# wolfbox/snappy

Hardware: AMD Instinct MI355X
Metric: GiB/s hashed (whole node), bit-exact hashes.yaml, 10k x 1 MiB tree (higher is better)
Workload: dtype u64; 1 GPU; C2: ONE on-disk tree (tmpfs) of 10001 files (10 000 x 1 MiB + the 1 MiB archive stand-in) -> hashes.yaml, sharded over 1 rank(s) on 1 distinct GPU(s); bytes=10486808576, kernel=sha512_split_kernel<true>, tree_home=/dev/shm

## Files before the change

snappy_amd/csrc/hostfill.cpp:

```cpp
#include "hostfill.h"

#include <new>

#include <ctype.h>
#include <dirent.h>
#include <errno.h>
#include <sched.h>
#include <stdio.h>
#include <string.h>
#include <sys/syscall.h>
#include <unistd.h>

#include <algorithm>
#include <atomic>

#if defined(__x86_64__)
#include <immintrin.h>
#endif

namespace snaphash {

namespace {

bool read_small_file(const std::string& path, std::string& out)
// ... 103 lines not shown
}

int numa_node_of_address(const void* addr)
{
#if defined(SYS_get_mempolicy)
    int node = -1;
    if (syscall(SYS_get_mempolicy, &node, nullptr, 0ul, addr, (unsigned long)(kMpolFNode | kMpolFAddr)) != 0) return -1;
    return node;
#else
    (void)addr;
    return -1;
#endif
}

unsigned cgroup_cpu_quota(const std::string& sysfs_cgroup_root, const std::string& proc_self_cgroup)
{
    std::string text;
    if (!read_small_file(proc_self_cgroup, text)) return 0;
    double best = 0;
    auto take = [&](double quota, double period) {
        if (quota > 0 && period > 0) { const double c = quota / period; if (best == 0 || c < best) best = c; }
    };
    size_t pos = 0;
    while (pos < text.size()) {
        size_t eol = text.find('\n', pos);
        if (eol == std::string::npos) eol = text.size();
        const std::string line = text.substr(pos, eol - pos);
        pos = eol + 1;
        const size_t c1 = line.find(':'), c2 = c1 == std::string::npos ? c1 : line.find(':', c1 + 1);
        if (c2 == std::string::npos) continue;
        const std::string ctrl = line.substr(c1 + 1, c2 - c1 - 1);
        std::string path = line.substr(c2 + 1);
        const bool v2 = ctrl.empty();
        if (!v2) {
            bool has_cpu = false;
            for (size_t a = 0; a <= ctrl.size();) {
                size_t b = ctrl.find(',', a);
                if (b == std::string::npos) b = ctrl.size();
                if (ctrl.compare(a, b - a, "cpu") == 0) has_cpu = true;
                a = b + 1;
            }
            if (!has_cpu) continue;
        }
        const std::string base = sysfs_cgroup_root + (v2 ? "" : "/" + ctrl);
        for (;;) {
            std::string v;
            if (v2) {
                if (read_small_file(base + path + "/cpu.max", v) && v.compare(0, 3, "max") != 0) {
                    char* end = nullptr;
                    const double q = strtod(v.c_str(), &end);
                    const double per = end ? strtod(end, nullptr) : 0;
                    take(q, per);
                }
            } else {
                std::string pv;
                if (read_small_file(base + path + "/cpu.cfs_quota_us", v) && read_small_file(base + path + "/cpu.cfs_period_us", pv))
                    take(strtod(v.c_str(), nullptr), strtod(pv.c_str(), nullptr));
            }
            if (path.empty() || path == "/") break;
            const size_t slash = path.rfind('/');
            path = slash == 0 || slash == std::string::npos ? "/" : path.substr(0, slash);
        }
    }
    if (best <= 0) return 0;
    return (unsigned)std::max(1.0, best + 0.5);
}

unsigned usable_cpus()
{
    unsigned n = 0;
    cpu_set_t set;
    CPU_ZERO(&set);
    if (sched_getaffinity(0, sizeof set, &set) == 0) {
        const int c = CPU_COUNT(&set);
        if (c > 0) n = (unsigned)c;
    }
    if (n == 0) n = std::max(1u, std::thread::hardware_concurrency());
    static const unsigned quota = cgroup_cpu_quota("/sys/fs/cgroup", "/proc/self/cgroup");
    if (quota && quota < n) n = quota;
    return n;
}


FillPool::~FillPool() { stop(); }

void FillPool::stop()
{
    {
        std::lock_guard<std::mutex> lk(mu_);
        quit_ = true;
    }
    cv_work_.notify_all();
    for (auto& t : th_) if (t.joinable()) t.join();
    th_.clear();
    quit_ = false;
}

void FillPool::configure(unsigned max_threads, const std::vector<int>& cpus)
{
    stop();
    max_threads_ = max_threads;
    cpus_ = cpus;
}

void FillPool::worker(unsigned id)
{
    if (!cpus_.empty()) {
        cpu_set_t set, allowed;
        CPU_ZERO(&set);
        CPU_ZERO(&allowed);
        const bool have_allowed = sched_getaffinity(0, sizeof allowed, &allowed) == 0;
        for (int c : cpus_)
            if (c >= 0 && c < CPU_SETSIZE && (!have_allowed || CPU_ISSET(c, &allowed))) CPU_SET(c, &set);
        if (CPU_COUNT(&set) > 0) (void)sched_setaffinity(0, sizeof set, &set);
    }
    uint64_t seen = 0;
    for (;;) {
        const std::function<void(size_t)>* fn;
        size_t n;
        std::atomic<size_t>* next;
        {
            std::unique_lock<std::mutex> lk(mu_);
            cv_work_.wait(lk, [&] { return quit_ || (epoch_ != seen && id < want_); });
            if (quit_) return;
            seen = epoch_;
            fn = fn_; n = n_; next = next_;
        }
        try {
            for (;;) {
                const size_t i = next->fetch_add(1);
                if (i >= n) break;
                (*fn)(i);
            }
        } catch (...) {
            fn_threw_.store(true);
        }
        {
            std::lock_guard<std::mutex> lk(mu_);
            if (--running_ == 0) cv_done_.notify_all();
        }
    }
}

void FillPool::parallel_for(size_t n, unsigned threads, const std::function<void(size_t)>& fn)
{
    if (n == 0) return;
    unsigned helpers = threads > 1 ? std::min(threads - 1, max_threads_) : 0u;
    if (helpers > n - 1) helpers = (unsigned)(n - 1);
    std::atomic<size_t> next{0};
    if (helpers) {
        std::lock_guard<std::mutex> lk(mu_);
        try {
            while (th_.size() < helpers) { const unsigned id = (unsigned)th_.size(); th_.emplace_back(&FillPool::worker, this, id); }
        } catch (...) {
            helpers = (unsigned)th_.size();
        }
        if (helpers) {
            fn_ = &fn; n_ = n; next_ = &next;
            want_ = helpers;
            running_ = helpers;
            ++epoch_;
        }
    }
    if (helpers) cv_work_.notify_all();
    bool threw = false;
    try {
        for (;;) {
            const size_t i = next.fetch_add(1);
            if (i >= n) break;
            fn(i);
        }
    } catch (...) {
        threw = true;
        next.store(n);
    }
    if (helpers) {
        std::unique_lock<std::mutex> lk(mu_);
        cv_done_.wait(lk, [&] { return running_ == 0; });
        want_ = 0;
        fn_ = nullptr; next_ = nullptr;
    }
    if (fn_threw_.exchange(false) || threw) throw std::bad_alloc();
}


void run_on_threads(unsigned T, const std::function<void(unsigned)>& fn)
{
    if (T <= 1) { fn(0); return; }
    static std::mutex mu;
    static FillPool* pool = [] {
        FillPool* p = new FillPool();
        p->configure(64, {});
        return p;
    }();
    static const pid_t born_in = getpid();
    if (T <= 65 && getpid() == born_in && mu.try_lock()) {
        std::lock_guard<std::mutex> lk(mu, std::adopt_lock);
        pool->parallel_for(T, T, [&fn](size_t t) { fn((unsigned)t); });
// ... 41 lines not shown
```

snappy_amd/csrc/hostfill.h:

```cpp
#pragma once
#include <stddef.h>
#include <stdint.h>

#include <atomic>
#include <condition_variable>
#include <functional>
#include <mutex>
#include <new>
#include <string>
#include <thread>
#include <vector>

namespace snaphash {

int numa_node_of_pci(const std::string& sysfs_root, const std::string& bdf);
std::vector<int> numa_cpus_of_node(const std::string& sysfs_root, int node);
std::vector<int> parse_cpulist(const std::string& text);
int numa_node_count(const std::string& sysfs_root);
std::vector<int> slice_cpus(const std::vector<int>& all, size_t pos, size_t m);

struct SavedMemPolicy {
    bool valid = false;
    int mode = 0;
    unsigned long mask[1024 / (8 * sizeof(unsigned long)) + 1] = {0};
};
bool numa_prefer_node(int node, SavedMemPolicy* saved);
void numa_restore_policy(const SavedMemPolicy& saved);
int numa_node_of_address(const void* addr);
unsigned usable_cpus();
unsigned cgroup_cpu_quota(const std::string& sysfs_cgroup_root, const std::string& proc_self_cgroup);

struct ThreadJoiner {
    std::vector<std::thread> th;
    std::atomic<bool> worker_threw{false};
    ThreadJoiner() = default;
    ThreadJoiner(const ThreadJoiner&) = delete;
    ThreadJoiner& operator=(const ThreadJoiner&) = delete;
    ~ThreadJoiner() { join_quietly(); }
    template <class F, class... A> void spawn(F&& f, A&&... a)
    {
        th.emplace_back([this](auto fn, auto... args) {
            try { fn(args...); } catch (...) { worker_threw.store(true); }
        }, std::forward<F>(f), std::forward<A>(a)...);
    }
    void join_quietly()
    {
        for (auto& t : th)
            if (t.joinable()) t.join();
    }
    void join_all()
    {
        join_quietly();
        if (worker_threw.exchange(false)) throw std::bad_alloc();
    }
};

class FillPool {
public:
    FillPool() = default;
    ~FillPool();
    FillPool(const FillPool&) = delete;
    FillPool& operator=(const FillPool&) = delete;
    void configure(unsigned max_threads, const std::vector<int>& cpus);
    void parallel_for(size_t n, unsigned threads, const std::function<void(size_t)>& fn);
    unsigned max_threads() const { return max_threads_; }
    const std::vector<int>& cpus() const { return cpus_; }

private:
    void worker(unsigned id);
    void stop();
    unsigned max_threads_ = 0;
    std::vector<int> cpus_;
    std::vector<std::thread> th_;
    std::mutex mu_;
    std::condition_variable cv_work_, cv_done_;
    uint64_t epoch_ = 0;
    unsigned want_ = 0;
    unsigned running_ = 0;
    bool quit_ = false;
    const std::function<void(size_t)>* fn_ = nullptr;
    std::atomic<bool> fn_threw_{false};
    size_t n_ = 0;
    std::atomic<size_t>* next_ = nullptr;
};

void run_on_threads(unsigned T, const std::function<void(unsigned)>& fn);

void copy_to_staging(void* dst, const void* src, size_t n);

}
```

snappy_amd/csrc/snaphash_api.cpp:

```cpp
#include <dirent.h>
#include <errno.h>
#include <fcntl.h>
#include <hip/hip_runtime.h>
#include <string.h>
#include <sys/resource.h>
#include <sys/stat.h>
#include <unistd.h>

#include <algorithm>
#include <atomic>
#include <queue>
#include <chrono>
#include <string>
#include <thread>
#include <unordered_map>
#include <vector>

#include <dlfcn.h>
#include <rccl/rccl.h>

#include <condition_variable>
#include <functional>
#include <future>
#include <memory>
#include <mutex>

#include "batchplan.h"
#include "engine_bufs.h"
#include "hostfill.h"
#include "hostpass.h"
#include "hostsha.h"
#include "inflate_host.h"
#include "member_hashers.h"
#include "planner.h"
#include "sha512_core.h"
#include "sha512_kernels.h"
#include "snap_core.h"
#include "tarpack.h"
#include "walk.h"

using namespace snaphash;

namespace {

constexpr uint64_t kDefaultStaging = 256ull << 20;

struct EventPair { hipEvent_t a = nullptr, b = nullptr; int kind = 0; };

double now_ms()
{
    using namespace std::chrono;
    return duration<double, std::milli>(steady_clock::now().time_since_epoch()).count();
}

}

struct snaphash_ctx;

struct DevCtx {
    int device = 0;
    int index = 0;
    hipStream_t stream = nullptr;
    bool own_stream = false;
    hipStream_t copy_stream = nullptr;
    uint64_t staging = kDefaultStaging;
    uint32_t kernel_pref = SNAPHASH_KERNEL_AUTO;
    uint32_t deflate_depth = 0;
    uint32_t n_xcd = 8;

    std::vector<SubSlot> sub;
    Slot slot[3];
    HashBufs hash;
    Twin<CmpChunk> cmp;
    DeflateBufs z;
    hipStream_t z_stream = nullptr;
    hipStream_t z2_stream = nullptr;
    std::vector<hipEvent_t> z_ev;
    std::vector<hipEvent_t> z_part_ev;
    InflateBufs inf;
    Bzip2Bufs bz;
    CrcBufs crc;
    XzBufs xz;
    hipStream_t f_stream = nullptr;
    uint64_t fout_gen = 0;

    std::vector<EventPair> ev_pool;
    size_t ev_used = 0;
    bool pending = false;

    std::string pci_bus_id;
    int numa_node = -1;
    int staging_node = -1;
    int64_t fd_budget = 0;
    int64_t fd_call_budget = -1;
    unsigned fill_cap = 12;
    unsigned fill_call_cap = 0;
    snaphash_ctx* owner = nullptr;
    unsigned owner_cpus_per_engine = 0;
    uint64_t staged_calls = 0;
    double fill_thread_s = 0;
    uint64_t fill_bytes = 0;
    FillPool pool;

    snaphash_stats stats{};
    double t_call0 = 0;
    std::string last_error;

    template <class F> void each_buf(F&& f)
    {
        for (Slot& s : slot) s.each(f);
        for (SubSlot& q : sub) q.jobs.each(f);
        hash.each(f);
        cmp.each(f);
        z.each(f);
        inf.each(f);
        bz.each(f);
        crc.each(f);
        xz.each(f);
    }
};

namespace {
struct Rccl {
    void* lib = nullptr;
    bool tried = false, ok = false;
    std::string why;
    ncclResult_t (*CommInitAll)(ncclComm_t*, int, const int*) = nullptr;
    ncclResult_t (*CommDestroy)(ncclComm_t) = nullptr;
    ncclResult_t (*AllGather)(const void*, void*, size_t, ncclDataType_t, ncclComm_t, hipStream_t) = nullptr;
    ncclResult_t (*GroupStart)() = nullptr;
    ncclResult_t (*GroupEnd)() = nullptr;
    const char* (*GetErrorString)(ncclResult_t) = nullptr;
    std::vector<ncclComm_t> comms;
};
}

struct snaphash_batch;

struct snaphash_ctx {
    std::vector<std::unique_ptr<DevCtx>> dev;
    uint32_t host_threads = 0;
    bool gpu_only = false;
    unsigned cpus = 1;
    unsigned cpus_call = 0;
    double host_rate = 1.4e9;
    PlanCalib calib;
    std::mutex calib_mu;
    uint32_t flags = 0;
    Rccl rccl;
    std::vector<DevBuf<uint8_t>> d_gather;
    snaphash_stats stats{};
    snaphash_stats_ex ex{};
    snaphash_targz_stats targz{};
    snaphash_unpack_stats unpack{};
    snaphash_block_scan_stats block_scan{};
    std::string last_error;
    snaphash_batch* open_batch = nullptr;
    DevCtx* d0() const { return dev[0].get(); }
};

namespace {

int fail(DevCtx* c, int code, const std::string& msg)
{
    if (c) c->last_error = msg;
    return code;
}
int fail(snaphash_ctx* x, int code, const std::string& msg)
{
    if (x) x->last_error = msg;
    return code;
}
int lift(snaphash_ctx* x, DevCtx* c, int rc)
{
    if (rc && x && c) x->last_error = c->last_error;
    return rc;
}
#define HIP_TRY(c, expr)                                                                             \
    do {                                                                                             \
        hipError_t e_ = (expr);                                                                      \
        if (e_ != hipSuccess)                                                                        \
            return fail(c, (e_ == hipErrorOutOfMemory) ? SNAPHASH_ENOMEM : SNAPHASH_EDEVICE,         \
                        std::string(#expr) + ": " + hipGetErrorString(e_));                          \
    } while (0)

// ... 24 lines not shown
            (void)hipEventElapsedTime(&t1, c->ev_pool[0].a, c->ev_pool[i].b);
            fprintf(stderr, "snaphash engine %d: %s %7.2f .. %7.2f ms\n", c->index, c->ev_pool[i].kind == 0 ? "kernel" : c->ev_pool[i].kind == 1 ? "h2d   " : "other ", t0, t1);
        }
    }
    c->ev_used = 0;
}

}

hipError_t snaphash::devbuf_alloc(Mem kind, void** p, size_t bytes, int numa_node)
{
    if (kind == Mem::Hbm) return hipMalloc(p, bytes);
    SavedMemPolicy saved;
    if (numa_node >= 0 && numa_prefer_node(numa_node, &saved)) {
        const hipError_t e = hipHostMalloc(p, bytes, hipHostMallocNumaUser);
        numa_restore_policy(saved);
        if (e == hipSuccess) return e;
        (void)hipGetLastError();
    }
    return hipHostMalloc(p, bytes, hipHostMallocDefault);
}

void snaphash::devbuf_free(Mem kind, void* p)
{
    if (kind == Mem::Hbm) (void)hipFree(p);
    else (void)hipHostFree(p);
}

namespace {

int ensure_slots(DevCtx* c, int nslots = 2, uint64_t want = 0)
{
    if (want == 0 || want > c->staging) want = c->staging;
    for (int k = 0; k < nslots; ++k) {
        Slot& s = c->slot[k];
        HIP_TRY(c, s.ensure(want, c->numa_node));
        if (c->staging_node < 0) { s.h_buf[0] = 0; c->staging_node = numa_node_of_address(s.h_buf.data()); }
        if (!s.done) HIP_TRY(c, hipEventCreateWithFlags(&s.done, hipEventDisableTiming));
        if (!s.copied) HIP_TRY(c, hipEventCreateWithFlags(&s.copied, hipEventDisableTiming));
    }
    if (!c->copy_stream) HIP_TRY(c, hipStreamCreateWithFlags(&c->copy_stream, hipStreamNonBlocking));
    return SNAPHASH_OK;
}

constexpr size_t kSplitMaxStreams = 32768;
constexpr uint64_t kSplitMinBlocks = 32;

uint64_t job_blocks(const Job& j) { return (j.nbytes >> 7) + 1; }

hipError_t launch_kernel(uint32_t k, const Job* d_jobs, size_t n, DevCtx* c, uint8_t* d_digests, bool staged)
{
    if (k == SNAPHASH_KERNEL_QUAD) return launch_quad(d_jobs, (uint32_t)n, c->hash.d_state.data(), d_digests, c->stream);
    if (k == SNAPHASH_KERNEL_PAIR) return launch_pair(d_jobs, (uint32_t)n, c->hash.d_state.data(), d_digests, c->stream, staged);
    if (k == SNAPHASH_KERNEL_SPLIT) return launch_split(d_jobs, (uint32_t)n, c->hash.d_state.data(), d_digests, c->stream);
    return launch_wide(d_jobs, (uint32_t)n, c->hash.d_state.data(), d_digests, c->stream);
}

size_t plan_kernels(const DevCtx* c, const Job* h_jobs, size_t n, uint32_t* k_head, uint32_t* k_tail)
{
    *k_tail = SNAPHASH_KERNEL_WIDE;
    if (c->kernel_pref == SNAPHASH_KERNEL_WIDE || c->kernel_pref == SNAPHASH_KERNEL_SPLIT ||
        c->kernel_pref == SNAPHASH_KERNEL_PAIR || c->kernel_pref == SNAPHASH_KERNEL_QUAD) {
        *k_head = c->kernel_pref;
        return n;
    }
    *k_head = SNAPHASH_KERNEL_PAIR;
    uint64_t blocks = 0;
    for (size_t i = 0; i < n; ++i) blocks += job_blocks(h_jobs[i]);
    if (n <= kSplitMaxStreams) {
        if (blocks >= kSplitMinBlocks * n) return n;
        *k_head = SNAPHASH_KERNEL_WIDE;
        return n;
    }
    if (job_blocks(h_jobs[0]) >= 8 * job_blocks(h_jobs[kSplitMaxStreams - 1]) &&
        job_blocks(h_jobs[0]) >= kSplitMinBlocks) {
        size_t head = 0;
        while (head < kSplitMaxStreams && job_blocks(h_jobs[head]) >= kSplitMinBlocks) ++head;
        return head;
    }
    *k_head = SNAPHASH_KERNEL_WIDE;
    return n;
}

int launch_jobs(DevCtx* c, Job* h_jobs, Job* d_jobs, size_t n, uint8_t* d_digests, hipEvent_t copied = nullptr)
{
    if (n == 0) return SNAPHASH_OK;
    std::stable_sort(h_jobs, h_jobs + n, [](const Job& a, const Job& b) { return a.nbytes > b.nbytes; });
    if (copied) {
        HIP_TRY(c, hipMemcpyAsync(d_jobs, h_jobs, n * sizeof(Job), hipMemcpyHostToDevice, c->copy_stream));
        HIP_TRY(c, hipEventRecord(copied, c->copy_stream));
        HIP_TRY(c, hipStreamWaitEvent(c->stream, copied, 0));
    } else {
        HIP_TRY(c, hipMemcpyAsync(d_jobs, h_jobs, n * sizeof(Job), hipMemcpyHostToDevice, c->stream));
    }
    uint32_t k_head, k_tail;
    const size_t head = plan_kernels(c, h_jobs, n, &k_head, &k_tail);
    EventPair* ev = next_events(c, 0);
    if (!ev) return fail(c, SNAPHASH_EDEVICE, "hipEventCreate failed");
    HIP_TRY(c, hipEventRecord(ev->a, c->stream));
    const bool staged = copied != nullptr;
    hipError_t e = launch_kernel(k_head, d_jobs, head, c, d_digests, staged);
    if (e == hipSuccess && head < n) e = launch_kernel(k_tail, d_jobs + head, n - head, c, d_digests, staged);
    if (e != hipSuccess) return fail(c, SNAPHASH_EDEVICE, std::string("kernel launch: ") + hipGetErrorString(e));
    HIP_TRY(c, hipEventRecord(ev->b, c->stream));
    c->stats.launches += (head < n) ? 2 : 1;
    c->stats.kernel_used = k_head;
    c->pending = true;
    return SNAPHASH_OK;
}

int sync_ctx(DevCtx* c)
{
    if (!c->pending && c->ev_used == 0) return SNAPHASH_OK;
    if (c->copy_stream) HIP_TRY(c, hipStreamSynchronize(c->copy_stream));
    HIP_TRY(c, hipStreamSynchronize(c->stream));
    collect_events(c);
    c->pending = false;
    if (c->t_call0 > 0) { c->stats.wall_ms = now_ms() - c->t_call0; c->t_call0 = 0; }
    return SNAPHASH_OK;
}

void begin_call(DevCtx* c)
{
    c->stats = snaphash_stats{};
    c->t_call0 = now_ms();
    c->last_error.clear();
}


struct FdCache {
    std::vector<int> fd;
    std::atomic<int64_t> held{0};
    int64_t budget = 0;
    explicit FdCache(size_t n, int64_t b) : fd(n, -1), budget(b) {}
    ~FdCache() { for (int f : fd) if (f >= 0) close(f); }
    FdCache(const FdCache&) = delete;
    FdCache& operator=(const FdCache&) = delete;
};

int do_read_op(const Source& s, const ReadOp& op, FdCache* cache = nullptr)
{
    if (s.mem) { copy_to_staging(op.dst, s.mem + op.off, op.n); return 0; }
    int err = 0;
    int fd = cache ? cache->fd[op.src] : -1;
    bool cached = fd >= 0;
    if (fd < 0) {
        for (unsigned tries = 0;; ++tries) {
            fd = open(s.path, O_RDONLY | O_CLOEXEC);
            if (fd >= 0 || (errno != EMFILE && errno != ENFILE) || tries >= 2000) break;
            usleep(tries < 100 ? 200 : 2000);
        }
        if (fd < 0) err = errno;
        else if (cache && !op.to_eof && cache->held.load(std::memory_order_relaxed) < cache->budget) {
            cache->fd[op.src] = fd;
            cache->held.fetch_add(1, std::memory_order_relaxed);
            cached = true;
        }
    }
    uint64_t got = 0;
    while (!err && got < op.n) {
        ssize_t r = pread(fd, op.dst + got, op.n - got, (off_t)(op.off + got));
        if (r < 0) { if (errno == EINTR) continue; err = errno; }
        else if (r == 0) err = EIO;
        else got += (uint64_t)r;
    }
    if (!err && op.to_eof) {
        uint8_t probe;
        ssize_t r;
        do r = pread(fd, &probe, 1, (off_t)(op.off + op.n)); while (r < 0 && errno == EINTR);
        if (r > 0) err = EIO;
        else if (r < 0) err = errno;
    }
    if (fd >= 0 && (!cached || op.to_eof || err)) {
        close(fd);
        if (cached) { cache->fd[op.src] = -1; cache->held.fetch_sub(1, std::memory_order_relaxed); }
    }
    return err;
}

void run_reads(DevCtx* c, const std::vector<Source>& src, const std::vector<ReadOp>& ops, std::atomic<int>& first_err,
               std::atomic<int64_t>& first_err_src, FdCache* cache = nullptr, bool alone = false)
{
    static const int forced = [] {
        const char* e = getenv("SNAPHASH_COPY_THREADS");
        const int v = e ? atoi(e) : 0;
        return (v >= 1 && v <= 256) ? v : 0;
    }();
    const bool from_memory = !ops.empty() && src[ops[0].src].mem != nullptr;
    unsigned cap = forced ? (unsigned)forced : std::min(c->fill_cap, from_memory ? 6u : 12u);
    if (!forced && c->fill_call_cap) cap = std::min(cap, c->fill_call_cap);
    if (!forced && alone && !c->fill_call_cap && c->owner) cap = std::max(cap, std::min(c->fill_cap * 2u, c->owner_cpus_per_engine));
    const unsigned T = (unsigned)std::min<size_t>(cap, std::max<size_t>(1, ops.size() / 4));
    const double t_fill0 = now_ms();
    struct FillAccount {
        DevCtx* c; const std::vector<ReadOp>& ops; unsigned T; double t0;
        ~FillAccount()
        {
            uint64_t b = 0;
            for (const ReadOp& op : ops) b += op.n;
            c->fill_bytes += b;
            c->fill_thread_s += (now_ms() - t0) * 1e-3 * T;
        }
    } account{c, ops, T, t_fill0};
    c->pool.parallel_for(ops.size(), T, [&](size_t i) {
        if (first_err.load(std::memory_order_relaxed)) return;
        const ReadOp& op = ops[i];
        const int err = do_read_op(src[op.src], op, cache);
        if (err) {
            int z = 0;
            if (first_err.compare_exchange_strong(z, err)) first_err_src.store(op.src);
        }
    });
}

struct EngineSpans { float gpu = 0, copy_busy = 0, copy = 0; };
EngineSpans engine_spans(DevCtx* c)
{
    EngineSpans sp;
    if (c->copy_stream) (void)hipStreamSynchronize(c->copy_stream);
    (void)hipStreamSynchronize(c->stream);
    size_t first_copy = c->ev_used, last_copy = 0, last_kernel = 0;
    for (size_t i = 0; i < c->ev_used; ++i) {
        float ms = 0;
        if (c->ev_pool[i].kind == 1) {
            if (first_copy == c->ev_used) first_copy = i;
            last_copy = i;
            if (hipEventElapsedTime(&ms, c->ev_pool[i].a, c->ev_pool[i].b) == hipSuccess) sp.copy_busy += ms;
        } else if (c->ev_pool[i].kind == 0) last_kernel = i;
    }
    if (first_copy < c->ev_used) {
        (void)hipEventElapsedTime(&sp.gpu, c->ev_pool[first_copy].a, c->ev_pool[last_kernel].b);
        (void)hipEventElapsedTime(&sp.copy, c->ev_pool[first_copy].a, c->ev_pool[last_copy].b);
    }
    return sp;
}

int hash_sources(DevCtx* c, const std::vector<Source>& src, uint8_t* digests, uint64_t* states, int* err_no,
                 int64_t* err_src)
{
    const size_t n = src.size();
    if (err_no) *err_no = 0;
    if (err_src) *err_src = -1;
    if (n == 0) return SNAPHASH_OK;
    HIP_TRY(c, hipSetDevice(c->device));
    uint64_t job_bytes = 0;
    for (const Source& sc : src) job_bytes += sc.gpu_len;
    const bool from_memory = src[0].mem != nullptr;
    const uint64_t slot_caps[3] = {c->slot[0].cap(), c->slot[1].cap(), c->slot[2].cap()};
    const BatchGeometry g = batch_geometry(job_bytes, n, c->staging, slot_caps, from_memory);
    int rc = ensure_slots(c, (int)g.nslots, g.slot_bytes);
    if (rc) return rc;
    HIP_TRY(c, c->hash.ensure(n, true));
    if (c->sub.size() < g.nsub) c->sub.resize(g.nsub);
    for (unsigned q = 0; q < g.nsub; ++q) {
        SubSlot& ss = c->sub[q];
        if (!ss.done) HIP_TRY(c, hipEventCreateWithFlags(&ss.done, hipEventDisableTiming));
        if (!ss.copied) HIP_TRY(c, hipEventCreateWithFlags(&ss.copied, hipEventDisableTiming));
        ss.busy = false;
    }

    c->fill_thread_s = 0;
    c->fill_bytes = 0;
    BatchPlanner plan(src.data(), n, job_bytes, g.S_full, BatchKnobs::from_env());
    std::atomic<int> first_err{0};
    std::atomic<int64_t> first_err_src{-1};
    std::vector<ReadOp> ops;
    FdCache fds(from_memory ? 0 : n, c->fd_call_budget >= 0 ? std::min(c->fd_call_budget, c->fd_budget) : c->fd_budget);
    double t_wait = 0, t_plan = 0, t_read = 0, t_launch = 0;
    const double t_engine0 = now_ms();
    double t_first_copy = 0;
    size_t n_copies = 0;

    while (!plan.active.empty()) {
        const unsigned batch = plan.batch, q = batch % g.nsub;
        SubSlot& sl = c->sub[q];
        uint8_t* const sl_h = c->slot[q / g.per_slot].h_buf.data() + (uint64_t)(q % g.per_slot) * g.S_full;
        uint8_t* const sl_d = c->slot[q / g.per_slot].d_buf.data() + (uint64_t)(q % g.per_slot) * g.S_full;
        const double tb0 = now_ms();
        if (sl.busy) { HIP_TRY(c, hipEventSynchronize(sl.done)); sl.busy = false; }
        const double tb1 = now_ms();
        t_wait += tb1 - tb0;
        HIP_TRY(c, sl.jobs.ensure(plan.active.size()));
        const Batch b = plan.next(sl.jobs.h.data(), ops, (uint64_t)(uintptr_t)sl_h, (uint64_t)(uintptr_t)sl_d);
        c->stats.blocks += b.blocks;
        static const bool trace_batches = getenv("SNAPHASH_TRACE_BATCHES") != nullptr;
        if (trace_batches) trace_batch(stderr, c->index, batch, b, sl.jobs.h.data(), (uint64_t)(uintptr_t)sl_d, plan.active.size());
        const double tb2 = now_ms();
        t_plan += tb2 - tb1;

        run_reads(c, src, ops, first_err, first_err_src, from_memory ? nullptr : &fds, batch == 0);
        if (first_err.load()) break;
        const double tb3 = now_ms();
        t_read += tb3 - tb2;
        if (trace_batches)
            fprintf(stderr, "snaphash engine %d: batch %u: at %.2f ms: waited %.2f, planned %.2f, filled %.2f ms (%zu streams begun, %.1f GB/s)\n", c->index, batch,
                    tb0 - t_engine0, tb1 - tb0, tb2 - tb1, tb3 - tb2, b.n_new, (double)b.used / ((tb3 - tb2) * 1e6 + 1e-9));

        if (b.used) {
            if (batch == 0) t_first_copy = now_ms() - t_engine0;
            ++n_copies;
            EventPair* ev = next_events(c, 1);
            if (!ev) return fail(c, SNAPHASH_EDEVICE, "hipEventCreate failed");
            HIP_TRY(c, hipEventRecord(ev->a, c->copy_stream));
            HIP_TRY(c, hipMemcpyAsync(sl_d, sl_h, b.used, hipMemcpyHostToDevice, c->copy_stream));
            HIP_TRY(c, hipEventRecord(ev->b, c->copy_stream));
        }
        rc = launch_jobs(c, sl.jobs.h.data(), sl.jobs.d.data(), b.nj, c->hash.d_digests.data(), sl.copied);
        if (rc) return rc;
        HIP_TRY(c, hipEventRecord(sl.done, c->stream));
        sl.busy = true;
        t_launch += now_ms() - tb3;
    }

    const double ts0 = now_ms();
    static const bool trace_tree = getenv("SNAPHASH_TRACE_TREE") != nullptr;
    const EngineSpans sp = trace_tree && c->ev_used > 1 ? engine_spans(c) : EngineSpans{};
    rc = sync_ctx(c);
    if (trace_tree)
        fprintf(stderr, "snaphash engine %d: %u batches; waiting for a slot %.1f ms, planning %.1f ms, reads %.1f ms, enqueue %.1f ms, drain %.1f ms; "
                        "first copy enqueued at %.2f ms, copies busy %.2f of %.2f ms, first copy -> last kernel %.2f ms, engine %.2f ms\n",
                c->index, plan.batch, t_wait, t_plan, t_read, t_launch, now_ms() - ts0, t_first_copy, sp.copy_busy, sp.copy, sp.gpu, now_ms() - t_engine0);
    for (SubSlot& ss : c->sub) ss.busy = false;
    if (rc) return rc;
    if (first_err.load()) {
        const int64_t s = first_err_src.load();
        if (err_no) *err_no = first_err.load();
        if (err_src) *err_src = s;
        return fail(c, SNAPHASH_EIO,
                    std::string(s >= 0 && src[s].path ? src[s].path : "<buffer>") + ": " + strerror(first_err.load()));
    }
    if (digests) HIP_TRY(c, hipMemcpy(digests, c->hash.d_digests.data(), n * 64, hipMemcpyDeviceToHost));
    if (states) HIP_TRY(c, hipMemcpy(states, c->hash.d_state.data(), n * 64, hipMemcpyDeviceToHost));
    for (size_t i = 0; i < n; ++i) c->stats.bytes_hashed += src[i].gpu_len;
    c->stats.streams = n;
    if (c->owner) {
        std::lock_guard<std::mutex> lk(c->owner->calib_mu);
        const double planned = c->owner->ex.planned_gpu_ms, took = now_ms() - t_engine0;
        const bool take_fill = c->staged_calls++ > 0 && !(planned > 0 && took > 3.0 * planned);
        c->owner->calib.observe_call(!from_memory, (double)c->fill_bytes, (double)n, (double)n_copies, c->stats.h2d_ms * 1e-3, c->fill_thread_s, take_fill);
    }
    return SNAPHASH_OK;
}


bool rccl_load(snaphash_ctx* x)
{
    Rccl& r = x->rccl;
    if (r.tried) return r.ok;
    r.tried = true;
    for (const char* name : {"librccl.so.1", "librccl.so", "/opt/rocm/lib/librccl.so.1"}) {
        r.lib = dlopen(name, RTLD_NOW | RTLD_LOCAL);
        if (r.lib) break;
    }
    if (!r.lib) { r.why = "librccl.so not found"; return false; }
    r.CommInitAll = (decltype(r.CommInitAll))dlsym(r.lib, "ncclCommInitAll");
    r.CommDestroy = (decltype(r.CommDestroy))dlsym(r.lib, "ncclCommDestroy");
    r.AllGather = (decltype(r.AllGather))dlsym(r.lib, "ncclAllGather");
    r.GroupStart = (decltype(r.GroupStart))dlsym(r.lib, "ncclGroupStart");
    r.GroupEnd = (decltype(r.GroupEnd))dlsym(r.lib, "ncclGroupEnd");
    r.GetErrorString = (decltype(r.GetErrorString))dlsym(r.lib, "ncclGetErrorString");
    if (!r.CommInitAll || !r.CommDestroy || !r.AllGather || !r.GroupStart || !r.GroupEnd) {
        r.why = "librccl.so lacks a required symbol";
        return false;
    }
    std::vector<int> devs;
    for (auto& d : x->dev) devs.push_back(d->device);
    std::vector<int> uniq = devs;
    std::sort(uniq.begin(), uniq.end());
    if (std::adjacent_find(uniq.begin(), uniq.end()) != uniq.end()) {
        r.why = "a device ordinal repeats in the ctx (RCCL needs one rank per GPU)";
        return false;
    }
    r.comms.assign(devs.size(), nullptr);
    const ncclResult_t e = r.CommInitAll(r.comms.data(), (int)devs.size(), devs.data());
    if (e != ncclSuccess) {
        r.why = std::string("ncclCommInitAll: ") + (r.GetErrorString ? r.GetErrorString(e) : "error");
        r.comms.clear();
        return false;
    }
    r.ok = true;
    return true;
}

int gather_digest_slabs(snaphash_ctx* x, const std::vector<size_t>& cnt, size_t kmax, std::vector<uint8_t>& rows)
{
    const size_t nd = x->dev.size();
    rows.assign(nd * kmax * 64, 0);
    const double t0 = now_ms();
    bool use_rccl = !(x->flags & SNAPHASH_FLAG_NO_RCCL) && rccl_load(x);
    if (use_rccl) {
        x->d_gather.resize(nd);
        for (size_t d = 0; d < nd; ++d) {
            DevCtx* c = x->dev[d].get();
            HIP_TRY(c, hipSetDevice(c->device));
            if (x->d_gather[d].reserve(nd * kmax * 64) != hipSuccess)
                return fail(x, SNAPHASH_ENOMEM, "hipMalloc of the gather buffer failed");
            HIP_TRY(x, c->hash.ensure(kmax, true));
        }
        Rccl& r = x->rccl;
        ncclResult_t e = r.GroupStart();
        for (size_t d = 0; d < nd && e == ncclSuccess; ++d) {
            DevCtx* c = x->dev[d].get();
            (void)hipSetDevice(c->device);
            e = r.AllGather(c->hash.d_digests.data(), x->d_gather[d].data(), kmax * 64, ncclUint8, r.comms[d], c->stream);
// ... 499 lines not shown
    const unsigned ncpu = usable_cpus();
    x->cpus = ncpu;
    if (v2) {
        x->flags = cfg->flags;
        x->host_threads = std::min<uint32_t>(cfg->host_threads, 256);
    }
    if (!cfg && getenv("SNAPHASH_HOST_THREADS")) {
        x->host_threads = (uint32_t)std::min<unsigned long>(strtoul(getenv("SNAPHASH_HOST_THREADS"), nullptr, 10), 256);
        if (x->host_threads == 0) x->flags |= SNAPHASH_FLAG_GPU_ONLY;
    }
    x->gpu_only = (x->flags & SNAPHASH_FLAG_GPU_ONLY) != 0;
    if (!x->gpu_only) x->host_rate = measure_host_rate();
    const char* sysfs_env = getenv("SNAPHASH_SYSFS_ROOT");
    const std::string sysfs = sysfs_env && *sysfs_env ? sysfs_env : "/sys";
    const bool numa_on = !(x->flags & SNAPHASH_FLAG_NO_NUMA) && numa_node_count(sysfs) > 1;
    const unsigned fill_cap = std::max(2u, std::min(12u, ncpu / (unsigned)devs.size()));
    int64_t fd_budget = 0;
    {
        struct rlimit rl;
        if (getrlimit(RLIMIT_NOFILE, &rl) == 0) {
            const rlim_t want = rl.rlim_max == RLIM_INFINITY ? 65536 : std::min<rlim_t>(rl.rlim_max, 65536);
            const bool keep = (cfg && cfg->struct_size >= sizeof(snaphash_config) && (cfg->flags & SNAPHASH_FLAG_KEEP_RLIMIT)) || getenv("SNAPHASH_KEEP_RLIMIT");
            if (!keep && rl.rlim_cur != RLIM_INFINITY && rl.rlim_cur < want) {
                struct rlimit up = rl;
                up.rlim_cur = want;
                if (setrlimit(RLIMIT_NOFILE, &up) == 0) rl = up;
            }
            const int64_t soft = rl.rlim_cur == RLIM_INFINITY ? 65536 : (int64_t)rl.rlim_cur;
            fd_budget = std::max<int64_t>(0, std::min<int64_t>(soft - 512, 32768)) / (int64_t)devs.size();
        }
    }
    for (size_t k = 0; k < devs.size(); ++k) {
        const int dev = devs[k];
        if (dev < 0 || dev >= ndev) {
            for (auto& d : x->dev) destroy_dev(d.get());
            return init_fail(SNAPHASH_EINVAL, "device ordinal out of range");
        }
        hipDeviceProp_t prop;
        int rc = SNAPHASH_OK;
        std::string why;
        if ((e = hipGetDeviceProperties(&prop, dev)) != hipSuccess) { rc = SNAPHASH_EDEVICE; why = "hipGetDeviceProperties"; }
        else if (strncmp(prop.gcnArchName, "gfx950", 6) != 0) {
            rc = SNAPHASH_EDEVICE;
            e = hipSuccess;
            why = std::string("device is ") + prop.gcnArchName + ", this library is built for gfx950 only";
        } else if ((e = hipSetDevice(dev)) != hipSuccess) { rc = SNAPHASH_EDEVICE; why = "hipSetDevice"; }
        std::unique_ptr<DevCtx> c(rc ? nullptr : new (std::nothrow) DevCtx());
        if (!rc && !c) rc = SNAPHASH_ENOMEM;
        if (!rc) {
            c->device = dev;
            c->index = (int)k;
            if (v1) {
                if (cfg->staging_bytes) c->staging = (cfg->staging_bytes + kAlign - 1) & ~(uint64_t)(kAlign - 1);
                c->kernel_pref = cfg->kernel;
                if (cfg->deflate_depth) c->deflate_depth = std::min<uint32_t>(std::max<uint32_t>(cfg->deflate_depth, 4u), 256u) & ~3u;
                if (c->kernel_pref == SNAPHASH_KERNEL_QUAD && !have_quad_kernel()) {
                    rc = SNAPHASH_EINVAL;
                    e = hipSuccess;
                    why = "SNAPHASH_KERNEL_QUAD is not in this build (make QUAD=1)";
                }
                if (cfg->stream) c->stream = (hipStream_t)cfg->stream;
            }
        }
        if (!rc) {
            if (c->staging < (1u << 16)) c->staging = 1u << 16;
            c->fill_cap = fill_cap;
            c->fd_budget = fd_budget;
            if (!cfg && getenv("SNAPHASH_DEFLATE_DEPTH"))
                c->deflate_depth = std::min<uint32_t>(std::max<uint32_t>((uint32_t)strtoul(getenv("SNAPHASH_DEFLATE_DEPTH"), nullptr, 10), 4u), 256u) & ~3u;
            {
                int xcc = 0;
                if (hipDeviceGetAttribute(&xcc, hipDeviceAttributeNumberOfXccs, dev) == hipSuccess && xcc >= 1 && xcc <= 64) c->n_xcd = (uint32_t)xcc;
                else (void)hipGetLastError();
            }
            std::vector<int> cpus;
            char bdf[64] = {0};
            if (hipDeviceGetPCIBusId(bdf, (int)sizeof bdf, dev) == hipSuccess) c->pci_bus_id = bdf;
            else (void)hipGetLastError();
            if (numa_on) {
                c->numa_node = numa_node_of_pci(sysfs, c->pci_bus_id);
                cpus = numa_cpus_of_node(sysfs, c->numa_node);
            }
            c->pool.configure(256, cpus);
            if (!c->stream) {
                if ((e = hipStreamCreateWithFlags(&c->stream, hipStreamNonBlocking)) != hipSuccess) { rc = SNAPHASH_EDEVICE; why = "hipStreamCreateWithFlags"; }
                else c->own_stream = true;
            }
        }
        if (rc) {
            for (auto& d : x->dev) destroy_dev(d.get());
            return init_fail(rc, why, e);
        }
        x->dev.push_back(std::move(c));
    }
    if (numa_on && x->dev.size() > 1) {
        for (size_t k = 0; k < x->dev.size(); ++k) {
            DevCtx* c = x->dev[k].get();
            if (c->numa_node < 0) continue;
            size_t m = 0, pos = 0;
            for (size_t j = 0; j < x->dev.size(); ++j)
                if (x->dev[j]->numa_node == c->numa_node) { if (j == k) pos = m; ++m; }
            if (m < 2) continue;
            const std::vector<int> mine = slice_cpus(numa_cpus_of_node(sysfs, c->numa_node), pos, m);
            if (!mine.empty()) c->pool.configure(256, mine);
        }
    }
    for (auto& d : x->dev) { d->owner = x.get(); d->owner_cpus_per_engine = std::max(1u, ncpu / (unsigned)x->dev.size()); }
    if (!x->gpu_only) calibrate_at_init(x.get());
    *out = x.release();
    return SNAPHASH_OK;
} catch (...) {
    return SNAPHASH_ENOMEM;
}

void snaphash_destroy(snaphash_ctx* x)
{
    if (!x) return;
    if (x->open_batch) snaphash_batch_abort(x->open_batch);
    for (size_t d = 0; d < x->d_gather.size(); ++d)
        if (x->d_gather[d].data()) { (void)hipSetDevice(x->dev[d]->device); x->d_gather[d].reset(); }
    if (x->rccl.ok)
        for (ncclComm_t c : x->rccl.comms) if (c) (void)x->rccl.CommDestroy(c);
    for (auto& d : x->dev) destroy_dev(d.get());
    delete x;
}

#define TOP_ENTER(x)                                                                  \
    if ((x)->open_batch) return fail((x), SNAPHASH_EINVAL, "a streaming batch is open on this ctx"); \
    for (auto& d_ : (x)->dev) {                                                       \
        (void)hipSetDevice(d_->device);                                               \
        int rc_ = sync_ctx(d_.get());                                                 \
        if (rc_) return lift((x), d_.get(), rc_);                                     \
    }                                                                                 \
    begin_top(x);                                                                     \
    const double t_top0_ = now_ms()

int snaphash_sha512_files(snaphash_ctx* x, const char* const* paths, size_t n, uint8_t* digests, int32_t* status)
try {
    if (!x || (n && (!paths || !digests))) return fail(x, SNAPHASH_EINVAL, "bad argument");
    TOP_ENTER(x);
    int rc = hash_paths(x, paths, n, nullptr, digests, status);
    end_top(x, t_top0_);
    return rc;
} catch (...) {
    return SNAPHASH_ENOMEM;
}

int snaphash_sha512_buffers(snaphash_ctx* x, const void* const* bufs, const uint64_t* lens, size_t n, uint8_t* digests)
try {
    if (!x || (n && (!bufs || !lens || !digests))) return fail(x, SNAPHASH_EINVAL, "bad argument");
    TOP_ENTER(x);
    std::vector<Source> src(n);
    for (size_t i = 0; i < n; ++i) {
        if (!bufs[i] && lens[i]) return fail(x, SNAPHASH_EINVAL, "NULL buffer with non-zero length");
        src[i].mem = bufs[i] ? (const uint8_t*)bufs[i] : (const uint8_t*)"";
        src[i].len = lens[i];
    }
    int rc = hash_sources_top(x, src, digests, nullptr);
    end_top(x, t_top0_);
    return rc;
} catch (...) {
    return SNAPHASH_ENOMEM;
}

int snaphash_sha512_device(snaphash_ctx* x, const void* d_base, const uint64_t* offsets, const uint64_t* lens,
                           size_t n, void* d_digests)
try {
    if (!x || (n && (!d_base || !offsets || !lens || !d_digests))) return fail(x, SNAPHASH_EINVAL, "bad argument");
    if (((uintptr_t)d_base & 15) != 0) return fail(x, SNAPHASH_EINVAL, "d_base must be 16-byte aligned");
    if (n > 0xffffffffull) return fail(x, SNAPHASH_EINVAL, "too many streams");
    if (x->open_batch) return fail(x, SNAPHASH_EINVAL, "a streaming batch is open on this ctx");
    DevCtx* c = x->d0();
    HIP_TRY(c, hipSetDevice(c->device));
    int rc = sync_ctx(c);
    if (rc) return lift(x, c, rc);
    begin_top(x);
    begin_call(c);
    if (n == 0) return SNAPHASH_OK;
    HIP_TRY(x, c->hash.ensure(n, false, n));
    for (size_t i = 0; i < n; ++i) {
        if (offsets[i] & 15) return fail(x, SNAPHASH_EINVAL, "offsets must be 16-byte aligned");
        if (lens[i] >> 35) return fail(x, SNAPHASH_EINVAL, "a resident stream is limited to 32 GiB per call (32-bit block counters)");
        Job& j = c->hash.jobs.h[i];
        j.data = (uint64_t)(uintptr_t)d_base + offsets[i];
        j.nbytes = lens[i];
        j.total_prev = 0;
        j.idx = (uint32_t)i;
// ... 1395 lines not shown
```

Before: 50.18 GiB/s.

## Plan batches ahead on a helper thread and inline job tables into data copy

Adds a helper thread that plans the next batch (slot wait, planning, job sort, kernel choice) and pre-opens files while the main thread reads and launches the current batch, using a two-item handoff pipe. The job table is appended to the staging buffer so it travels in the same host-to-device copy instead of a separate memcpy. The goal is to take planning, open syscalls and slot waits off the critical read path. The cost is extra thread synchronisation and more complex error handling. The path is on by default and can be disabled with an environment variable.

```diff
diff --git a/snappy_amd/csrc/engine_pipe.h b/snappy_amd/csrc/engine_pipe.h
--- /dev/null
+++ b/snappy_amd/csrc/engine_pipe.h
@@ -0,0 +1,180 @@
+#pragma once
+#include <stddef.h>
+#include <stdlib.h>
+
+#include <condition_variable>
+#include <functional>
+#include <mutex>
+#include <thread>
+#include <utility>
+#include <vector>
+
+#include "batchplan.h"
+
+namespace snaphash {
+
+class PipeHelper {
+public:
+    PipeHelper() = default;
+    ~PipeHelper() { quit(); }
+    PipeHelper(const PipeHelper&) = delete;
+    PipeHelper& operator=(const PipeHelper&) = delete;
+    void configure(std::function<void()> at_start)
+    {
+        quit();
+        at_start_ = std::move(at_start);
+    }
+    bool run(std::function<void()> task)
+    {
+        std::unique_lock<std::mutex> lk(mu_);
+        if (!th_.joinable()) {
+            try { th_ = std::thread(&PipeHelper::loop, this); } catch (...) { return false; }
+        }
+        task_ = std::move(task);
+        busy_ = true;
+        lk.unlock();
+        cv_.notify_all();
+        return true;
+    }
+    void wait()
+    {
+        std::unique_lock<std::mutex> lk(mu_);
+        cv_.wait(lk, [&] { return !busy_; });
+    }
+    bool parked()
+    {
+        std::lock_guard<std::mutex> lk(mu_);
+        return !busy_;
+    }
+
+private:
+    void loop()
+    {
+        if (at_start_) at_start_();
+        std::unique_lock<std::mutex> lk(mu_);
+        for (;;) {
+            cv_.wait(lk, [&] { return quit_ || busy_; });
+            if (quit_) return;
+            std::function<void()> task = std::move(task_);
+            lk.unlock();
+            task();
+            task = nullptr;
+            lk.lock();
+            busy_ = false;
+            cv_.notify_all();
+        }
+    }
+    void quit()
+    {
+        {
+            std::unique_lock<std::mutex> lk(mu_);
+            cv_.wait(lk, [&] { return !busy_; });
+            quit_ = true;
+        }
+        cv_.notify_all();
+        if (th_.joinable()) th_.join();
+        quit_ = false;
+    }
+    std::mutex mu_;
+    std::condition_variable cv_;
+    std::thread th_;
+    std::function<void()> at_start_, task_;
+    bool busy_ = false, quit_ = false;
+};
+
+template <class Item> class BatchPipe {
+public:
+    BatchPipe(PipeHelper& helper, std::function<bool(unsigned, Item&)> produce) : helper_(helper), produce_(std::move(produce)) {}
+    ~BatchPipe() { stop(); }
+    BatchPipe(const BatchPipe&) = delete;
+    BatchPipe& operator=(const BatchPipe&) = delete;
+
+    Item item[2];
+
+    bool start()
+    {
+        started_ = helper_.run([this] { produce_all(); });
+        return started_;
+    }
+    Item* take()
+    {
+        std::unique_lock<std::mutex> lk(mu_);
+        cv_.wait(lk, [&] { return published_ > taken_ || finished_; });
+        if (published_ == taken_) return nullptr;
+        Item* it = &item[taken_ & 1];
+        ++taken_;
+        lk.unlock();
+        cv_.notify_all();
+        return it;
+    }
+    void stop()
+    {
+        if (!started_) return;
+        {
+            std::lock_guard<std::mutex> lk(mu_);
+            stop_ = true;
+        }
+        cv_.notify_all();
+        helper_.wait();
+        started_ = false;
+    }
+    bool threw()
+    {
+        std::lock_guard<std::mutex> lk(mu_);
+        return threw_;
+    }
+
+private:
+    void produce_all()
+    {
+        bool threw = false;
+        try {
+            for (unsigned k = 0;; ++k) {
+                {
+                    std::unique_lock<std::mutex> lk(mu_);
+                    cv_.wait(lk, [&] { return stop_ || taken_ >= k; });
+                    if (stop_) break;
+                }
+                if (!produce_(k, item[k & 1])) break;
+                {
+                    std::lock_guard<std::mutex> lk(mu_);
+                    published_ = k + 1;
+                }
+                cv_.notify_all();
+            }
+        } catch (...) {
+            threw = true;
+        }
+        {
+            std::lock_guard<std::mutex> lk(mu_);
+            finished_ = true;
+            threw_ = threw;
+        }
+        cv_.notify_all();
+    }
+    PipeHelper& helper_;
+    std::function<bool(unsigned, Item&)> produce_;
+    std::mutex mu_;
+    std::condition_variable cv_;
+    unsigned published_ = 0, taken_ = 0;
+    bool finished_ = false, stop_ = false, threw_ = false, started_ = false;
+};
+
+template <class Open> size_t for_each_file_begun(const std::vector<ReadOp>& ops, const Source* src, Open&& open)
+{
+    size_t n = 0;
+    for (const ReadOp& op : ops) {
+        if (op.off != 0 || src[op.src].mem) continue;
+        if (!open(op)) break;
+        ++n;
+    }
+    return n;
+}
+
+inline bool engine_pipeline_from_env()
+{
+    const char* e = getenv("SNAPHASH_ENGINE_PIPELINE");
+    return !e || atoi(e) != 0;
+}
+
+}
diff --git a/snappy_amd/csrc/hostfill.cpp b/snappy_amd/csrc/hostfill.cpp
--- a/snappy_amd/csrc/hostfill.cpp
+++ b/snappy_amd/csrc/hostfill.cpp
@@ -209,6 +209,18 @@
 }
 
 
+void bind_thread_to_cpus(const std::vector<int>& cpus)
+{
+    if (cpus.empty()) return;
+    cpu_set_t set, allowed;
+    CPU_ZERO(&set);
+    CPU_ZERO(&allowed);
+    const bool have_allowed = sched_getaffinity(0, sizeof allowed, &allowed) == 0;
+    for (int c : cpus)
+        if (c >= 0 && c < CPU_SETSIZE && (!have_allowed || CPU_ISSET(c, &allowed))) CPU_SET(c, &set);
+    if (CPU_COUNT(&set) > 0) (void)sched_setaffinity(0, sizeof set, &set);
+}
+
 FillPool::~FillPool() { stop(); }
 
 void FillPool::stop()
@@ -232,15 +244,7 @@
 
 void FillPool::worker(unsigned id)
 {
-    if (!cpus_.empty()) {
-        cpu_set_t set, allowed;
-        CPU_ZERO(&set);
-        CPU_ZERO(&allowed);
-        const bool have_allowed = sched_getaffinity(0, sizeof allowed, &allowed) == 0;
-        for (int c : cpus_)
-            if (c >= 0 && c < CPU_SETSIZE && (!have_allowed || CPU_ISSET(c, &allowed))) CPU_SET(c, &set);
-        if (CPU_COUNT(&set) > 0) (void)sched_setaffinity(0, sizeof set, &set);
-    }
+    bind_thread_to_cpus(cpus_);
     uint64_t seen = 0;
     for (;;) {
         const std::function<void(size_t)>* fn;
diff --git a/snappy_amd/csrc/hostfill.h b/snappy_amd/csrc/hostfill.h
--- a/snappy_amd/csrc/hostfill.h
+++ b/snappy_amd/csrc/hostfill.h
@@ -55,6 +55,8 @@
     }
 };
 
+void bind_thread_to_cpus(const std::vector<int>& cpus);
+
 class FillPool {
 public:
     FillPool() = default;
diff --git a/snappy_amd/csrc/snaphash_api.cpp b/snappy_amd/csrc/snaphash_api.cpp
--- a/snappy_amd/csrc/snaphash_api.cpp
+++ b/snappy_amd/csrc/snaphash_api.cpp
@@ -27,6 +27,7 @@
 
 #include "batchplan.h"
 #include "engine_bufs.h"
+#include "engine_pipe.h"
 #include "hostfill.h"
 #include "hostpass.h"
 #include "hostsha.h"
@@ -101,6 +102,7 @@
     double fill_thread_s = 0;
     uint64_t fill_bytes = 0;
     FillPool pool;
+    PipeHelper plan_helper;
 
     snaphash_stats stats{};
     double t_call0 = 0;
@@ -291,23 +293,11 @@
     return n;
 }
 
-int launch_jobs(DevCtx* c, Job* h_jobs, Job* d_jobs, size_t n, uint8_t* d_digests, hipEvent_t copied = nullptr)
-{
-    if (n == 0) return SNAPHASH_OK;
-    std::stable_sort(h_jobs, h_jobs + n, [](const Job& a, const Job& b) { return a.nbytes > b.nbytes; });
-    if (copied) {
-        HIP_TRY(c, hipMemcpyAsync(d_jobs, h_jobs, n * sizeof(Job), hipMemcpyHostToDevice, c->copy_stream));
-        HIP_TRY(c, hipEventRecord(copied, c->copy_stream));
-        HIP_TRY(c, hipStreamWaitEvent(c->stream, copied, 0));
-    } else {
-        HIP_TRY(c, hipMemcpyAsync(d_jobs, h_jobs, n * sizeof(Job), hipMemcpyHostToDevice, c->stream));
-    }
-    uint32_t k_head, k_tail;
-    const size_t head = plan_kernels(c, h_jobs, n, &k_head, &k_tail);
+int launch_sorted(DevCtx* c, const Job* d_jobs, size_t n, size_t head, uint32_t k_head, uint32_t k_tail, uint8_t* d_digests, bool staged)
+{
     EventPair* ev = next_events(c, 0);
     if (!ev) return fail(c, SNAPHASH_EDEVICE, "hipEventCreate failed");
     HIP_TRY(c, hipEventRecord(ev->a, c->stream));
-    const bool staged = copied != nullptr;
     hipError_t e = launch_kernel(k_head, d_jobs, head, c, d_digests, staged);
     if (e == hipSuccess && head < n) e = launch_kernel(k_tail, d_jobs + head, n - head, c, d_digests, staged);
     if (e != hipSuccess) return fail(c, SNAPHASH_EDEVICE, std::string("kernel launch: ") + hipGetErrorString(e));
@@ -316,6 +306,27 @@
     c->stats.kernel_used = k_head;
     c->pending = true;
     return SNAPHASH_OK;
+}
+
+void sort_jobs(Job* h_jobs, size_t n)
+{
+    std::stable_sort(h_jobs, h_jobs + n, [](const Job& a, const Job& b) { return a.nbytes > b.nbytes; });
+}
+
+int launch_jobs(DevCtx* c, Job* h_jobs, Job* d_jobs, size_t n, uint8_t* d_digests, hipEvent_t copied = nullptr)
+{
+    if (n == 0) return SNAPHASH_OK;
+    sort_jobs(h_jobs, n);
+    if (copied) {
+        HIP_TRY(c, hipMemcpyAsync(d_jobs, h_jobs, n * sizeof(Job), hipMemcpyHostToDevice, c->copy_stream));
+        HIP_TRY(c, hipEventRecord(copied, c->copy_stream));
+        HIP_TRY(c, hipStreamWaitEvent(c->stream, copied, 0));
+    } else {
+        HIP_TRY(c, hipMemcpyAsync(d_jobs, h_jobs, n * sizeof(Job), hipMemcpyHostToDevice, c->stream));
+    }
+    uint32_t k_head, k_tail;
+    const size_t head = plan_kernels(c, h_jobs, n, &k_head, &k_tail);
+    return launch_sorted(c, d_jobs, n, head, k_head, k_tail, d_digests, copied != nullptr);
 }
 
 int sync_ctx(DevCtx* c)
@@ -444,6 +455,170 @@
     return sp;
 }
 
+
+constexpr uint64_t kNoTable = ~0ull;
+
+struct PassClock {
+    double t_wait = 0, t_plan = 0, t_read = 0, t_launch = 0;
+    double t_engine0 = 0;
+    double t_first_copy = 0;
+    size_t n_copies = 0;
+    bool pipelined = false;
+    double t_helper = 0;
+    size_t opened_ahead = 0;
+    unsigned tables_inline = 0;
+};
+
+struct PlannedBatch {
+    unsigned batch = 0;
+    Batch b;
+    std::vector<ReadOp> ops;
+    SubSlot* sl = nullptr;
+    uint8_t *sl_h = nullptr, *sl_d = nullptr;
+    size_t head = 0;
+    uint32_t k_head = 0, k_tail = 0;
+    uint64_t table_at = kNoTable;
+    size_t opened = 0;
+    double waited = 0, planned = 0;
+    std::string trace;
+    int rc = SNAPHASH_OK;
+};
+
+size_t open_ahead(const std::vector<Source>& src, const std::vector<ReadOp>& ops, FdCache& cache)
+{
+    return for_each_file_begun(ops, src.data(), [&](const ReadOp& op) {
+        if (cache.fd[op.src] >= 0) return true;
+        if (cache.held.fetch_add(1, std::memory_order_relaxed) >= cache.budget) {
+            cache.held.fetch_sub(1, std::memory_order_relaxed);
+            return false;
+        }
+        const int fd = open(src[op.src].path, O_RDONLY | O_CLOEXEC);
+        if (fd < 0) {
+            const bool out_of_fds = errno == EMFILE || errno == ENFILE;
+            cache.held.fetch_sub(1, std::memory_order_relaxed);
+            return !out_of_fds;
+        }
+        cache.fd[op.src] = fd;
+        return true;
+    });
+}
+
+int plan_ahead(DevCtx* c, const std::vector<Source>& src, const BatchGeometry& g, BatchPlanner& plan, FdCache* fds, unsigned k, bool trace_batches,
+               PlannedBatch& pb)
+{
+    const unsigned batch = plan.batch, q = batch % g.nsub;
+    SubSlot& sl = c->sub[q];
+    pb.batch = batch;
+    pb.sl = &sl;
+    pb.sl_h = c->slot[q / g.per_slot].h_buf.data() + (uint64_t)(q % g.per_slot) * g.S_full;
+    pb.sl_d = c->slot[q / g.per_slot].d_buf.data() + (uint64_t)(q % g.per_slot) * g.S_full;
+    pb.table_at = kNoTable;
+    pb.opened = 0;
+    pb.trace.clear();
+    const double t0 = now_ms();
+    if (k == 0) HIP_TRY(c, hipSetDevice(c->device));
+    if (sl.busy) { HIP_TRY(c, hipEventSynchronize(sl.done)); sl.busy = false; }
+    const double t1 = now_ms();
+    HIP_TRY(c, sl.jobs.ensure(plan.active.size()));
+    Job* const jobs = sl.jobs.h.data();
+    pb.b = plan.next(jobs, pb.ops, (uint64_t)(uintptr_t)pb.sl_h, (uint64_t)(uintptr_t)pb.sl_d);
+    if (trace_batches) {
+        char* text = nullptr;
+        size_t len = 0;
+        if (FILE* f = open_memstream(&text, &len)) {
+            trace_batch(f, c->index, batch, pb.b, jobs, (uint64_t)(uintptr_t)pb.sl_d, plan.active.size());
+            fclose(f);
+            pb.trace.assign(text, len);
+            free(text);
+        }
+    }
+    const size_t nj = pb.b.nj;
+    sort_jobs(jobs, nj);
+    pb.head = nj ? plan_kernels(c, jobs, nj, &pb.k_head, &pb.k_tail) : 0;
+    const uint64_t at = (pb.b.used + kAlign - 1) & ~(uint64_t)(kAlign - 1);
+    if (nj && at + nj * sizeof(Job) <= g.S_full) {
+        memcpy(pb.sl_h + at, jobs, nj * sizeof(Job));
+        pb.table_at = at;
+    }
+    if (fds && k > 0) pb.opened = open_ahead(src, pb.ops, *fds);
+    pb.waited = t1 - t0;
+    pb.planned = now_ms() - t1;
+    return SNAPHASH_OK;
+}
+
+int run_pipelined(DevCtx* c, const std::vector<Source>& src, const BatchGeometry& g, BatchPlanner& plan, FdCache* fds, std::atomic<int>& first_err,
+                  std::atomic<int64_t>& first_err_src, PassClock& pc, bool* ran)
+{
+    static const bool trace_batches = getenv("SNAPHASH_TRACE_BATCHES") != nullptr;
+    bool helper_failed = false;
+    BatchPipe<PlannedBatch> pipe(c->plan_helper, [&](unsigned k, PlannedBatch& pb) {
+        if (helper_failed || plan.active.empty() || first_err.load()) return false;
+        pb.rc = plan_ahead(c, src, g, plan, fds, k, trace_batches, pb);
+        helper_failed = pb.rc != SNAPHASH_OK;
+        return true;
+    });
+    *ran = pipe.start();
+    if (!*ran) return SNAPHASH_OK;
+    pc.pipelined = true;
+    for (;;) {
+        const double tb0 = now_ms();
+        PlannedBatch* const pb = pipe.take();
+        const double tb2 = now_ms();
+        pc.t_helper += tb2 - tb0;
+        if (!pb) break;
+        if (pb->rc) return pb->rc;
+        const Batch& b = pb->b;
+        SubSlot& sl = *pb->sl;
+        c->stats.blocks += b.blocks;
+        pc.t_wait += pb->waited;
+        pc.t_plan += pb->planned;
+        pc.opened_ahead += pb->opened;
+        if (trace_batches) fputs(pb->trace.c_str(), stderr);
+
+        run_reads(c, src, pb->ops, first_err, first_err_src, fds, pb->batch == 0);
+        if (first_err.load()) break;
+        const double tb3 = now_ms();
+        pc.t_read += tb3 - tb2;
+        if (trace_batches)
+            fprintf(stderr, "snaphash engine %d: batch %u: at %.2f ms: waited %.2f, planned %.2f, filled %.2f ms (%zu streams begun, %.1f GB/s); the helper's wait and plan, %zu opens ahead; took it after %.2f ms\n",
+                    c->index, pb->batch, tb0 - pc.t_engine0, pb->waited, pb->planned, tb3 - tb2, b.n_new, (double)b.used / ((tb3 - tb2) * 1e6 + 1e-9), pb->opened, tb2 - tb0);
+
+        const bool table_inline = pb->table_at != kNoTable;
+        const uint64_t up = table_inline ? pb->table_at + b.nj * sizeof(Job) : b.used;
+        if (up) {
+            EventPair* ev = nullptr;
+            if (b.used) {
+                if (pb->batch == 0) pc.t_first_copy = now_ms() - pc.t_engine0;
+                ++pc.n_copies;
+                ev = next_events(c, 1);
+                if (!ev) return fail(c, SNAPHASH_EDEVICE, "hipEventCreate failed");
+                HIP_TRY(c, hipEventRecord(ev->a, c->copy_stream));
+            }
+            HIP_TRY(c, hipMemcpyAsync(pb->sl_d, pb->sl_h, up, hipMemcpyHostToDevice, c->copy_stream));
+            if (ev) HIP_TRY(c, hipEventRecord(ev->b, c->copy_stream));
+        }
+        const Job* d_jobs = sl.jobs.d.data();
+        if (table_inline) {
+            d_jobs = (const Job*)(pb->sl_d + pb->table_at);
+            ++pc.tables_inline;
+        } else if (b.nj) {
+            HIP_TRY(c, hipMemcpyAsync(sl.jobs.d.data(), sl.jobs.h.data(), b.nj * sizeof(Job), hipMemcpyHostToDevice, c->copy_stream));
+        }
+        if (b.nj) {
+            HIP_TRY(c, hipEventRecord(sl.copied, c->copy_stream));
+            HIP_TRY(c, hipStreamWaitEvent(c->stream, sl.copied, 0));
+            const int rc = launch_sorted(c, d_jobs, b.nj, pb->head, pb->k_head, pb->k_tail, c->hash.d_digests.data(), true);
+            if (rc) return rc;
+        }
+        HIP_TRY(c, hipEventRecord(sl.done, c->stream));
+        sl.busy = true;
+        pc.t_launch += now_ms() - tb3;
+    }
+    pipe.stop();
+    if (pipe.threw()) throw std::bad_alloc();
+    return SNAPHASH_OK;
+}
+
 int hash_sources(DevCtx* c, const std::vector<Source>& src, uint8_t* digests, uint64_t* states, int* err_no,
                  int64_t* err_src)
 {
@@ -475,12 +650,22 @@
     std::atomic<int64_t> first_err_src{-1};
     std::vector<ReadOp> ops;
     FdCache fds(from_memory ? 0 : n, c->fd_call_budget >= 0 ? std::min(c->fd_call_budget, c->fd_budget) : c->fd_budget);
-    double t_wait = 0, t_plan = 0, t_read = 0, t_launch = 0;
-    const double t_engine0 = now_ms();
-    double t_first_copy = 0;
-    size_t n_copies = 0;
-
-    while (!plan.active.empty()) {
+    PassClock pc;
+    pc.t_engine0 = now_ms();
+    double &t_wait = pc.t_wait, &t_plan = pc.t_plan, &t_read = pc.t_read, &t_launch = pc.t_launch, &t_first_copy = pc.t_first_copy;
+    const double t_engine0 = pc.t_engine0;
+    size_t& n_copies = pc.n_copies;
+
+    if (engine_pipeline_from_env() && g.nsub >= 2 && job_bytes + kAlign * n > 2 * g.S_full) {
+        bool ran = false;
+        rc = run_pipelined(c, src, g, plan, from_memory ? nullptr : &fds, first_err, first_err_src, pc, &ran);
+        if (rc) {
+            for (SubSlot& ss : c->sub) ss.busy = false;
+            return rc;
+        }
+    }
+
+    while (!pc.pipelined && !plan.active.empty()) {
         const unsigned batch = plan.batch, q = batch % g.nsub;
         SubSlot& sl = c->sub[q];
         uint8_t* const sl_h = c->slot[q / g.per_slot].h_buf.data() + (uint64_t)(q % g.per_slot) * g.S_full;
@@ -527,8 +712,10 @@
     rc = sync_ctx(c);
     if (trace_tree)
         fprintf(stderr, "snaphash engine %d: %u batches; waiting for a slot %.1f ms, planning %.1f ms, reads %.1f ms, enqueue %.1f ms, drain %.1f ms; "
-                        "first copy enqueued at %.2f ms, copies busy %.2f of %.2f ms, first copy -> last kernel %.2f ms, engine %.2f ms\n",
-                c->index, plan.batch, t_wait, t_plan, t_read, t_launch, now_ms() - ts0, t_first_copy, sp.copy_busy, sp.copy, sp.gpu, now_ms() - t_engine0);
+                        "first copy enqueued at %.2f ms, copies busy %.2f of %.2f ms, first copy -> last kernel %.2f ms, engine %.2f ms; "
+                        "pipeline %s: waited for the helper %.2f ms, %zu opens ahead, %u job tables in the data copy\n",
+                c->index, plan.batch, t_wait, t_plan, t_read, t_launch, now_ms() - ts0, t_first_copy, sp.copy_busy, sp.copy, sp.gpu, now_ms() - t_engine0,
+                pc.pipelined ? "on" : "off", pc.t_helper, pc.opened_ahead, pc.tables_inline);
     for (SubSlot& ss : c->sub) ss.busy = false;
     if (rc) return rc;
     if (first_err.load()) {
@@ -1194,6 +1381,7 @@
                 cpus = numa_cpus_of_node(sysfs, c->numa_node);
             }
             c->pool.configure(256, cpus);
+            c->plan_helper.configure([cpus] { bind_thread_to_cpus(cpus); });
             if (!c->stream) {
                 if ((e = hipStreamCreateWithFlags(&c->stream, hipStreamNonBlocking)) != hipSuccess) { rc = SNAPHASH_EDEVICE; why = "hipStreamCreateWithFlags"; }
                 else c->own_stream = true;
@@ -1214,7 +1402,10 @@
                 if (x->dev[j]->numa_node == c->numa_node) { if (j == k) pos = m; ++m; }
             if (m < 2) continue;
             const std::vector<int> mine = slice_cpus(numa_cpus_of_node(sysfs, c->numa_node), pos, m);
-            if (!mine.empty()) c->pool.configure(256, mine);
+            if (!mine.empty()) {
+                c->pool.configure(256, mine);
+                c->plan_helper.configure([mine] { bind_thread_to_cpus(mine); });
+            }
         }
     }
     for (auto& d : x->dev) { d->owner = x.get(); d->owner_cpus_per_engine = std::max(1u, ncpu / (unsigned)x->dev.size()); }
```

Result: no change. 50.20 GiB/s, median of 2 (+0.0%).
